# pvjosue/CWFA

Measured on AMD Instinct MI355X. Metric: volumes/sec inverse-pass @512×512×96 fp32; NLL match vs ref (1/2/4/8 GPU), higher is better.
Workload: dtype f32 (storage, accumulation, wavelets, couplings); convolution products on the bf16 matrix cores from an exact three-way bf16 split of both fp32 operands, six products per fp32 product: fp32-equivalent; plain-fp32-MFMA figure: fp32_mfma; 1 GPU; 512x512x96 volume, 4-scale CWFA (CAT blocks, 64 ch) + LRNN inverse, z=0, batch 1/GPU, random-init weights (BASELINE.json configs[2]); precision=split, parallelism=replicated x1 (independent volumes per GPU, no collective)

## Files before the change

### cwfa_amd/_lib.py

```python
import ctypes as C
import os

_HERE = os.path.dirname(os.path.abspath(__file__))
LIB_PATH = os.path.join(_HERE, "libcwfa_hip.so")

CLAMP = {"NONE": 0, "ATAN": 1, "TANH": 2, "SIGMOID": 3}
ACT = {None: 0, "none": 0, "elu": 1, "prelu": 2, "gelu": 3, "relu": 4}
CHAIN_MAX = 8

c_f32p = C.c_void_p
c_i64p = C.c_void_p
c_f64p = C.c_void_p


class AffineStage(C.Structure):
    _fields_ = [("s_raw", c_f32p), ("t", c_f32p), ("s_bs", C.c_int64), ("t_bs", C.c_int64), ("clamp_kind", C.c_int),
                ("clamp", C.c_float), ("pre_scale", C.c_float), ("t_neg_div_sqrt2", C.c_int), ("perm", c_i64p),
                ("perm_axis", C.c_int), ("gin", C.c_int)]


class Chain(C.Structure):
    _fields_ = [("n_stages", C.c_int), ("stage", AffineStage * CHAIN_MAX), ("src_c", C.c_void_p), ("src_h", C.c_void_p)]


class ChainGrads(C.Structure):
    _fields_ = [("ds", c_f32p * CHAIN_MAX), ("dt", c_f32p * CHAIN_MAX), ("ds_bs", C.c_int64 * CHAIN_MAX),
                ("dt_bs", C.c_int64 * CHAIN_MAX)]


class ConvOpts(C.Structure):
    _fields_ = [("bias", c_f32p), ("act", C.c_int), ("prelu_alpha", c_f32p), ("residual", c_f32p), ("res_bs", C.c_int64),
                ("act2", C.c_int), ("in_scale", c_f32p), ("in_shift", c_f32p), ("in_affine_bs", C.c_int), ("in_add", c_f32p),
                ("in_add_bs", C.c_int64), ("upshuffle2", C.c_int), ("in_blocked8", C.c_int), ("out_blocked8", C.c_int),
                ("in_cat", c_f32p), ("in_cat_bs", C.c_int64), ("in_cat_from", C.c_int), ("in_cat_c1", C.c_int), ("out_stats", c_f64p), ("prelu_per_channel", C.c_int),
                ("out_sample_stats", c_f64p)]


class Couple(C.Structure):
    _fields_ = [("x", c_f32p), ("y", c_f32p), ("x_bs", C.c_int64), ("y_bs", C.c_int64), ("n", C.c_int), ("clamp_kind", C.c_int),
                ("clamp", C.c_float), ("pre_scale", C.c_float), ("rev", C.c_int), ("logdet", c_f64p), ("in_blocked8", C.c_int)]


class EvalAffine(C.Structure):
    _fields_ = [("enabled", C.c_int), ("scale", C.c_float), ("std", C.c_float), ("mean", C.c_float)]


class EvalPost(C.Structure):
    _fields_ = [("normalize", C.c_int), ("threshold", C.c_int), ("norm_sub", C.c_float), ("norm_div", C.c_float),
                ("vol_min", C.c_float), ("lower", C.c_float), ("upper", C.c_float), ("clamp_value", C.c_float)]

# ... 244 lines not shown
```

### cwfa_amd/csrc/conv2d.hip

```cpp
#include "conv_internal.h"

#include <string.h>
#include <type_traits>

namespace {

template <int KS_, int CK_, int MT_, int NT_, int WM_, int WN_, int XV_ = 1>
struct Cfg {
    static constexpr int KS = KS_, CK = CK_, MT = MT_, NT = NT_, WM = WM_, WN = WN_;
    static constexpr int XV = XV_;
    static_assert(XV_ == 1 || (XV_ == 4 && KS_ == 1), "vector staging needs halo-free tiles");
    static constexpr int PAD = KS / 2;
    static constexpr int NTHREADS = 64 * WM * WN;
    static constexpr int CT = 32 * MT * WM;
    static constexpr int TR = NT * WN;
    static constexpr int TC = 32;
    static constexpr int XR = TR + KS - 1;
    static constexpr int XC = TC + KS - 1;
    static constexpr int XS = CK * XR * XC;
    static constexpr int XS_PAD = (XS + 3) & ~3;
    static constexpr int WS = KS * KS * CK * CT;
    static constexpr int XPT = (XS / XV + NTHREADS - 1) / NTHREADS;
    static constexpr int WPT = (WS / 4 + NTHREADS - 1) / NTHREADS;
    static constexpr int BUF = XS_PAD + WS;
// ... 195 lines not shown
        chunk_body(chunk & 1, chunk, T{}, F{});
        ++chunk;
    }
    chunk_body(chunk & 1, chunk, F{}, F{});
}

__device__ __forceinline__ float ldg_off(const float* base, unsigned byte_off) {
    asm volatile("" : "+v"(byte_off));
    return *reinterpret_cast<const float*>(reinterpret_cast<const char*>(base) + byte_off);
}
__device__ __forceinline__ void stg_off(float* base, unsigned byte_off, float v) {
    asm volatile("" : "+v"(byte_off));
    *reinterpret_cast<float*>(reinterpret_cast<char*>(base) + byte_off) = v;
}

enum { EPI_GENERIC = 0, EPI_NONE, EPI_ELU, EPI_RES_ELU, EPI_PRELU, EPI_RES_PRELU, EPI_GELU_RES, EPI_UP, EPI_NONE_BLK8, EPI_COUNT };

template <int EPI>
struct EpiTraits {
    static constexpr int ACT1 = EPI == EPI_ELU ? CWFA_ACT_ELU : EPI == EPI_PRELU ? CWFA_ACT_PRELU
                                : EPI == EPI_GELU_RES ? CWFA_ACT_GELU : CWFA_ACT_NONE;
    static constexpr bool RES = EPI == EPI_RES_ELU || EPI == EPI_RES_PRELU || EPI == EPI_GELU_RES;
    static constexpr int ACT2 = EPI == EPI_RES_ELU ? CWFA_ACT_ELU : EPI == EPI_RES_PRELU ? CWFA_ACT_PRELU : CWFA_ACT_NONE;
    static constexpr bool UP = EPI == EPI_UP;
};

template <class C, int EPI>
__device__ __forceinline__ void epilogue(const ConvParams& p, const Tile& t, f32x16 (&acc)[C::MT][C::NT]) {
    typedef EpiTraits<EPI> E;
    const int64_t HW = (int64_t)p.H * p.W;
    const int col = t.col0 + t.l31;
    float* yb = p.y + (int64_t)t.b * p.y_bs;
    if constexpr (EPI == EPI_GENERIC) {
        const float alpha = (p.o.prelu_alpha && (p.o.act == CWFA_ACT_PRELU || p.o.act2 == CWFA_ACT_PRELU)) ? *p.o.prelu_alpha : 0.f;
        const float* rb = p.o.residual ? p.o.residual + (int64_t)t.b * p.o.res_bs : nullptr;
        extern __shared__ __attribute__((aligned(16))) float smem[];
        __syncthreads();
        float* mine = smem + (threadIdx.x >> 6) * 1024 + (threadIdx.x & 63);
        for (int m = 0; m < C::MT; ++m)
// ... 7 lines not shown
                            for (int r = 0; r < 16; ++r) mine[r * 64] = acc[mm][nn][r];
                        }
                const int row = t.row0 + t.wn * C::NT + n;
                for (int r = 0; r < 16; ++r) {
                    const int co = t.ct * C::CT + (t.wm * C::MT + m) * 32 + cwfa_acc_row(r, t.kh);
                    if (co >= p.Cout || row >= p.H || col >= p.W) continue;
                    const int cb = p.o.upshuffle2 ? co >> 2 : co;
                    int64_t o;
                    if (p.o.upshuffle2) {
                        const int q = co & 3;
                        o = (int64_t)cb * (4 * HW) + (int64_t)(2 * row + (q >> 1)) * (2 * p.W) + 2 * col + (q & 1);
                    } else {
                        o = (int64_t)co * HW + (int64_t)row * p.W + col;
                    }
                    float v = cwfa_act(mine[r * 64] + (p.o.bias ? p.o.bias[cb] : 0.f), p.o.act, alpha);
                    if (rb) v += rb[o];
                    yb[o] = cwfa_act(v, p.o.act2, alpha);
                }
            }
    } else {
        float alpha = 0.f;
        if constexpr (E::ACT1 == CWFA_ACT_PRELU || E::ACT2 == CWFA_ACT_PRELU) alpha = *p.o.prelu_alpha;
        const float* rb = nullptr;
        if constexpr (E::RES) rb = p.o.residual + (int64_t)t.b * p.o.res_bs;
        if constexpr (E::UP) {
            const int W2 = 2 * p.W;
            const bool al = ((W2 | (int)(p.y_bs & 1)) & 1) == 0 && ((reinterpret_cast<uintptr_t>(p.y) & 7) == 0);
#pragma unroll
            for (int m = 0; m < C::MT; ++m)
#pragma unroll
                for (int g = 0; g < 4; ++g) {
                    const int co = t.ct * C::CT + (t.wm * C::MT + m) * 32 + 8 * g + 4 * t.kh;
                    if (co >= p.Cout) continue;
                    const int c = co >> 2;
                    const float bias = p.o.bias ? p.o.bias[c] : 0.f;
#pragma unroll
                    for (int n = 0; n < C::NT; ++n) {
                        const int row = t.row0 + t.wn * C::NT + n;
                        if (row >= p.H || col >= p.W) continue;
                        float* o = yb + (int64_t)c * (4 * HW) + (int64_t)(2 * row) * W2 + 2 * col;
                        const float v0 = acc[m][n][4 * g] + bias, v1 = acc[m][n][4 * g + 1] + bias;
                        const float v2 = acc[m][n][4 * g + 2] + bias, v3 = acc[m][n][4 * g + 3] + bias;
                        if (al) {
                            *reinterpret_cast<float2*>(o) = make_float2(v0, v1);
                            *reinterpret_cast<float2*>(o + W2) = make_float2(v2, v3);
                        } else {
                            o[0] = v0; o[1] = v1; o[W2] = v2; o[W2 + 1] = v3;
                        }
                    }
                }
        } else if constexpr (EPI == EPI_NONE_BLK8) {
#pragma unroll
            for (int m = 0; m < C::MT; ++m)
#pragma unroll
                for (int q = 0; q < 4; ++q) {
                    const int co = t.ct * C::CT + (t.wm * C::MT + m) * 32 + 8 * q + 4 * t.kh;
                    if (co >= p.Cout) continue;
                    const f32x4 b4 = p.o.bias ? *reinterpret_cast<const f32x4*>(p.o.bias + co) : f32x4{0.f, 0.f, 0.f, 0.f};
#pragma unroll
                    for (int n = 0; n < C::NT; ++n) {
                        const int row = t.row0 + t.wn * C::NT + n;
                        if (row >= p.H || col >= p.W) continue;
                        f32x4 v;
#pragma unroll
                        for (int i = 0; i < 4; ++i) v[i] = acc[m][n][4 * q + i] + b4[i];
// ... 167 lines not shown
struct Sel {
    int id, CT, CK;
};

Sel select_cfg(int ks, int Cout) {
    const int cls = Cout <= 32 ? 0 : (Cout <= 64 ? 1 : 2);
    if (ks == 3) return cls == 0 ? Sel{0, C3_32::CT, C3_32::CK} : cls == 1 ? Sel{1, C3_64::CT, C3_64::CK} : Sel{2, C3_128::CT, C3_128::CK};
    if (ks == 1) return cls == 0 ? Sel{3, C1_32::CT, C1_32::CK} : cls == 1 ? Sel{4, C1_64::CT, C1_64::CK} : Sel{5, C1_128::CT, C1_128::CK};
    if (ks == 7) return cls == 0 ? Sel{6, C7_32::CT, C7_32::CK} : Sel{7, C7_64::CT, C7_64::CK};
    return Sel{-1, 0, 0};
}

int classify_epilogue(const cwfa_conv_opts& o) {
    const bool res = o.residual != nullptr;
    if (o.out_blocked8) return EPI_NONE_BLK8;
    if (o.upshuffle2) return (!res && o.act == CWFA_ACT_NONE && o.act2 == CWFA_ACT_NONE) ? EPI_UP : EPI_GENERIC;
    if (!res && o.act2 == CWFA_ACT_NONE) {
        if (o.act == CWFA_ACT_NONE) return EPI_NONE;
        if (o.act == CWFA_ACT_ELU) return EPI_ELU;
        if (o.act == CWFA_ACT_PRELU) return EPI_PRELU;
    }
    if (res && o.act == CWFA_ACT_NONE && o.act2 == CWFA_ACT_ELU) return EPI_RES_ELU;
    if (res && o.act == CWFA_ACT_NONE && o.act2 == CWFA_ACT_PRELU) return EPI_RES_PRELU;
    if (res && o.act == CWFA_ACT_GELU && o.act2 == CWFA_ACT_NONE) return EPI_GELU_RES;
    return EPI_GENERIC;
}

template <class C>
int prepare(ConvParams& p, dim3& grid) {
    p.tiles_x = (p.W + C::TC - 1) / C::TC;
    p.tiles_y = (p.H + C::TR - 1) / C::TR;
// ... 19 lines not shown
    CWFA_LAUNCH_CHECK("cwfa_conv2d_f32");
    return CWFA_OK;
}

template <class C, unsigned ALLOWED, bool PRO>
int launch_sel(const ConvParams& p, int epi, hipStream_t st) {
    if (!(ALLOWED & (1u << epi)) && epi != EPI_NONE_BLK8) epi = EPI_GENERIC;
    switch (epi) {
        case EPI_NONE: if constexpr (ALLOWED & (1u << EPI_NONE)) return launch_epi<C, EPI_NONE, PRO>(p, st); break;
        case EPI_ELU: if constexpr (ALLOWED & (1u << EPI_ELU)) return launch_epi<C, EPI_ELU, PRO>(p, st); break;
        case EPI_RES_ELU: if constexpr (ALLOWED & (1u << EPI_RES_ELU)) return launch_epi<C, EPI_RES_ELU, PRO>(p, st); break;
        case EPI_PRELU: if constexpr (ALLOWED & (1u << EPI_PRELU)) return launch_epi<C, EPI_PRELU, PRO>(p, st); break;
        case EPI_RES_PRELU: if constexpr (ALLOWED & (1u << EPI_RES_PRELU)) return launch_epi<C, EPI_RES_PRELU, PRO>(p, st); break;
        case EPI_GELU_RES: if constexpr (ALLOWED & (1u << EPI_GELU_RES)) return launch_epi<C, EPI_GELU_RES, PRO>(p, st); break;
        case EPI_UP: if constexpr (ALLOWED & (1u << EPI_UP)) return launch_epi<C, EPI_UP, PRO>(p, st); break;
        case EPI_NONE_BLK8:
            if constexpr (ALLOWED & (1u << EPI_NONE_BLK8)) return launch_epi<C, EPI_NONE_BLK8, PRO>(p, st);
            cwfa_set_error("cwfa_conv2d_f32: out_blocked8 is built for the 1x1 kernels with more than 32 output channels");
            return CWFA_E_SHAPE;
        default: break;
    }
    return launch_epi<C, EPI_GENERIC, PRO>(p, st);
}

template <class C, unsigned ALLOWED, unsigned ALLOWED_PRO>
int launch(const ConvParams& p, int epi, hipStream_t st) {
    if (p.o.in_scale || p.o.in_add) return launch_sel<C, ALLOWED_PRO, true>(p, epi, st);
    return launch_sel<C, ALLOWED, false>(p, epi, st);
}

// ... 6 lines not shown

int fill_params(ConvParams& p, const char* name, const float* x, const float* w_packed, float* y, int B, int Cin, int H,
                int W, int Cout, int64_t x_bs, int64_t y_bs, const cwfa_conv_opts* opts) {
    CWFA_REQUIRE(B >= 0 && Cin > 0 && Cout > 0 && H >= 0 && W >= 0, CWFA_E_INVAL, "%s: bad size", name);
    if (B == 0 || H == 0 || W == 0) return 1;
    CWFA_REQUIRE(x && w_packed && y, CWFA_E_INVAL, "%s: null pointer", name);
    CWFA_REQUIRE(!opts || !opts->out_sample_stats, CWFA_E_INVAL, "%s: out_sample_stats is a feature of the few-channel cwfa_conv7x7_split_f32", name);
    CWFA_REQUIRE((int64_t)Cin * H * W < (1ll << 30) && (int64_t)Cout * H * W * (p.o.upshuffle2 ? 1 : 1) < (1ll << 30), CWFA_E_SHAPE, "%s: C*H*W exceeds the 32-bit byte offsets of a tile (2^30 elements per image)", name);
    CWFA_REQUIRE(cwfa_aligned16(w_packed), CWFA_E_ALIGN, "%s: packed weights must be 16-byte aligned", name);
    p.x = x; p.wp = w_packed; p.y = y;
    p.B = B; p.Cin = Cin; p.H = H; p.W = W; p.Cout = Cout;
    p.x_bs = x_bs; p.y_bs = y_bs;
    p.products = g_cwfa_operand == CwfaOperand::split3 ? 6 : 1;
    if (opts) p.o = *opts;
    CWFA_REQUIRE(!(p.o.in_scale && !p.o.in_shift), CWFA_E_INVAL, "%s: in_scale without in_shift", name);
    CWFA_REQUIRE(p.o.act >= 0 && p.o.act <= CWFA_ACT_RELU && p.o.act2 >= 0 && p.o.act2 <= CWFA_ACT_RELU, CWFA_E_INVAL,
                 "%s: bad activation", name);
    CWFA_REQUIRE(!((p.o.act == CWFA_ACT_PRELU || p.o.act2 == CWFA_ACT_PRELU) && !p.o.prelu_alpha), CWFA_E_INVAL,
                 "%s: PReLU without prelu_alpha", name);
    return CWFA_OK;
}

typedef Cfg<1, 16, 2, 4, 4, 2> CS;
constexpr int CS_XB = 3 * 2 * 8 * 32 * 16, CS_WB = 3 * 2 * 256 * 16, CS_BUFB = CS_XB + CS_WB;

__device__ __forceinline__ void split3(float v, unsigned short (&o)[3]) {
    const __bf16 a1 = (__bf16)v;
    const float r1 = v - (float)a1;
    const __bf16 a2 = (__bf16)r1;
    const float r2 = r1 - (float)a2;
// ... 263 lines not shown
    ConvParams& p = sp.c;
    CWFA_REQUIRE(!p.o.in_scale && !p.o.in_add, CWFA_E_INVAL, "cwfa_conv_split_f32: the load-side prologue belongs in cwfa_split_input_f32");
    CWFA_REQUIRE(!p.o.upshuffle2 || (ks == 1 && Cout % 4 == 0), CWFA_E_SHAPE, "cwfa_conv_split_f32: upshuffle2 needs ks=1, Cout=4*Co");
    CWFA_REQUIRE(!p.o.out_stats && !p.o.prelu_per_channel, CWFA_E_INVAL, "cwfa_conv_split_f32: out_stats / prelu_per_channel are features of cwfa_conv3x3_split_f32");
    p.nchunks = (Cin + 15) / 16;
    sp.ws = ws;
    sp.CG2 = 2 * p.nchunks;
    sp.ws_bs = (int64_t)3 * sp.CG2 * H * W * 16;
    CWFA_REQUIRE(sp.ws_bs + (int64_t)4 * H * W * 16 < (1ll << 31) && (int64_t)(p.nchunks * ks * ks + 2) * CS_WB < (1ll << 31), CWFA_E_SHAPE,
                 "cwfa_conv_split_f32: one sample's planes / one cout tile's weights must stay below 2 GiB");
    const int epi = classify_epilogue(p.o);
    hipStream_t st = (hipStream_t)stream;
    switch (epi) {
        case EPI_NONE: return launch_split<EPI_NONE>(sp, st);
        case EPI_UP: return launch_split<EPI_UP>(sp, st);
        default: return launch_split<EPI_GENERIC>(sp, st);
    }
}

int g_cwfa_wino_min_cout = 1;
int g_cwfa_wino_2d = 512;
CwfaOperand g_cwfa_operand = CwfaOperand::split3;

extern "C" int cwfa_set_option(const char* name, int value) {
    CWFA_REQUIRE(name, CWFA_E_INVAL, "cwfa_set_option: null name");
    if (strcmp(name, "winograd_min_cout") == 0) {
        g_cwfa_wino_min_cout = value;
        return CWFA_OK;
    }
    if (strcmp(name, "winograd_2d") == 0) {
// ... 80 lines not shown
    CWFA_REQUIRE(!(opts && opts->out_blocked8) || (ks == 1 && Cout % 8 == 0 && !opts->residual && opts->act == CWFA_ACT_NONE &&
                                                   opts->act2 == CWFA_ACT_NONE && !opts->upshuffle2 && !opts->in_scale && !opts->in_add &&
                                                   cwfa_aligned16(y) && (y_bs & 3) == 0 && (!opts->bias || cwfa_aligned16(opts->bias))),
                 CWFA_E_INVAL, "cwfa_conv2d_f32: out_blocked8 needs a plain 1x1 bank (bias only), Cout %% 8 == 0 and 16-byte aligned y / bias");
    const Sel s = select_cfg(ks, Cout);
    CWFA_REQUIRE(s.id >= 0, CWFA_E_SHAPE, "cwfa_conv2d_f32: kernel size %d not in {1,3,7}", ks);
    ConvParams p{};
    int rc = fill_params(p, "cwfa_conv2d_f32", x, w_packed, y, B, Cin, H, W, Cout, x_bs, y_bs, opts);
    if (rc) return rc < 0 ? rc : CWFA_OK;
    CWFA_REQUIRE(!p.o.upshuffle2 || (ks == 1 && Cout % 4 == 0), CWFA_E_SHAPE, "cwfa_conv2d_f32: upshuffle2 needs ks=1, Cout=4*Co");
    CWFA_REQUIRE(!p.o.out_stats && !p.o.prelu_per_channel, CWFA_E_INVAL, "cwfa_conv2d_f32: out_stats / prelu_per_channel are features of cwfa_conv3x3_split_f32");
    const int epi = classify_epilogue(p.o);
    hipStream_t st = (hipStream_t)stream;
    if (cwfa_wino_selected(ks, Cout)) return cwfa_wino_conv(x, w_packed, y, B, Cin, H, W, Cout, x_bs, y_bs, p.o, st);
    constexpr unsigned N = 1u << EPI_NONE, E = 1u << EPI_ELU, RE = 1u << EPI_RES_ELU, P = 1u << EPI_PRELU,
                       RP = 1u << EPI_RES_PRELU, G = 1u << EPI_GELU_RES, U = 1u << EPI_UP, K = 1u << EPI_NONE_BLK8;
    const bool v4 = ks == 1 && (W & 3) == 0 && (x_bs & 3) == 0 && (reinterpret_cast<uintptr_t>(x) & 15) == 0 &&
                    (!p.o.in_add || ((p.o.in_add_bs & 3) == 0 && (reinterpret_cast<uintptr_t>(p.o.in_add) & 15) == 0));
    if (v4) {
        switch (s.id) {
            case 3: return launch<C1v_32, N | P | G, P>(p, epi, st);
            case 4: return launch<C1v_64, N | RE | G | K, 0>(p, epi, st);
            default: return launch<C1v_128, N | U | K, U>(p, epi, st);
        }
    }
    switch (s.id) {
        case 0: return launch<C3_32, N | P | RP, 0>(p, epi, st);
        case 1: return launch<C3_64, N | E | P | RP, 0>(p, epi, st);
        case 2: return launch<C3_128, N | P, P>(p, epi, st);
        case 3: return launch<C1_32, N | P | G, P>(p, epi, st);
        case 4: return launch<C1_64, N | RE | G | K, 0>(p, epi, st);
        case 5: return launch<C1_128, N | U | K, U>(p, epi, st);
        case 6: return launch<C7_32, N, 0>(p, epi, st);
        default: return launch<C7_64, N, 0>(p, epi, st);
    }
}

extern "C" int cwfa_subnet_pack1x1_f32(const float* w, float* panel, void* stream) {
    CWFA_REQUIRE(w && panel, CWFA_E_INVAL, "cwfa_subnet_pack1x1_f32: null pointer");
    hipLaunchKernelGGL(pack1x1_kernel, dim3(16), dim3(256), 0, (hipStream_t)stream, w, panel);
    CWFA_LAUNCH_CHECK("cwfa_subnet_pack1x1_f32");
    return CWFA_OK;
}

extern "C" int cwfa_subnet_layer_tape_f32(const float* x, const float* w3_packed, const float* b3, const float* w1_panel,
                                          const float* b1, float* y, float* hidden, int B, int H, int W, int64_t x_bs, int64_t y_bs,
                                          int64_t hidden_bs, void* stream) {
// ... 36 lines not shown
```

### cwfa_amd/csrc/conv_split3x3.hip

```cpp
#include "conv_internal.h"

extern int g_cwfa_split_xcd_map;
extern int g_cwfa_split_rows16;

namespace {

constexpr int TR = 8, TC = 32;

template <int KS, int RPW = 4>
struct XG {
    static constexpr int TRW = 2 * RPW, NT = 2 * RPW;
    static constexpr int PAD = KS / 2, XR = TRW + 2 * PAD, XC = TC + 2 * PAD, NTAP = KS * KS;
    static constexpr int EPK = XR * XC;
    static constexpr int KHB = KS == 7 ? 8512 : RPW == 8 ? 9792 : 5440;
    static constexpr int XPB = 2 * KHB;
    static constexpr int XB = 3 * XPB;
    static constexpr bool SPECIAL = KS == 3 && RPW == 4;
    static constexpr int NEK = SPECIAL ? 2 : 3;
    static_assert(EPK * 16 <= KHB && KHB % 256 == 64 && 2 * EPK <= 512 * NEK, "staging entry map");
    static_assert(!SPECIAL || (EPK > 256 && EPK <= 384), "3x3 staging entry map");
    static_assert(KS == 3 || RPW == 4, "7x7: 8-row tiles");
};

template <int MPW, int KS = 3, int RPW = 4, int WM = 4>
// ... 856 lines not shown
    pack_bank(w, packed, Cout, Cin, ct_of(Cout), 9, (hipStream_t)stream);
    CWFA_LAUNCH_CHECK("cwfa_conv3x3_split_pack_f32");
    return CWFA_OK;
}

extern "C" int cwfa_conv3x3_split_f32(const float* x, const void* w_packed, float* y, int B, int Cin, int H, int W, int Cout,
                                      int64_t x_bs, int64_t y_bs, const cwfa_conv_opts* opts, void* stream) {
    CWFA_REQUIRE(B >= 0 && Cin > 0 && Cout > 0 && H >= 0 && W >= 0, CWFA_E_INVAL, "cwfa_conv3x3_split_f32: bad size");
    if (B == 0 || H == 0 || W == 0) return CWFA_OK;
    CWFA_REQUIRE(x && w_packed && y, CWFA_E_INVAL, "cwfa_conv3x3_split_f32: null pointer");
    CWFA_REQUIRE(cwfa_aligned16(w_packed), CWFA_E_ALIGN, "cwfa_conv3x3_split_f32: packed weights must be 16-byte aligned");
    SParams p{};
    p.x = x; p.wp = w_packed; p.y = y;
    p.B = B; p.Cin = Cin; p.H = H; p.W = W; p.Cout = Cout; p.x_bs = x_bs; p.y_bs = y_bs;
    if (opts) p.o = *opts;
    CWFA_REQUIRE(!p.o.upshuffle2 && !p.o.in_cat, CWFA_E_SHAPE, "cwfa_conv3x3_split_f32: upshuffle2 / in_cat are 1x1 features");
    CWFA_REQUIRE(!p.o.out_sample_stats, CWFA_E_INVAL, "cwfa_conv3x3_split_f32: out_sample_stats is a feature of the few-channel cwfa_conv7x7_split_f32");
    CWFA_REQUIRE(!p.o.in_blocked8 || (Cin % 8 == 0 && cwfa_aligned16(x) && (x_bs & 3) == 0 && !p.o.in_add), CWFA_E_ALIGN,
                 "cwfa_conv3x3_split_f32: blocked input needs Cin %% 8 == 0, 16-byte alignment and no added tensor");
    CWFA_REQUIRE(!p.o.out_blocked8 || (Cout % 8 == 0 && cwfa_aligned16(y) && (y_bs & 3) == 0 && !p.o.residual && p.o.act2 == CWFA_ACT_NONE &&
                                       (p.o.act == CWFA_ACT_NONE || p.o.act == CWFA_ACT_PRELU)),
                 CWFA_E_ALIGN, "cwfa_conv3x3_split_f32: blocked output needs Cout %% 8 == 0, 16-byte alignment and a bias / PReLU epilogue");
    CWFA_REQUIRE(!(p.o.in_scale && !p.o.in_shift), CWFA_E_INVAL, "cwfa_conv3x3_split_f32: in_scale without in_shift");
    CWFA_REQUIRE(!p.o.out_stats || (!p.o.out_blocked8 && !p.o.residual && p.o.act2 == CWFA_ACT_NONE &&
                                    (p.o.act == CWFA_ACT_NONE || p.o.act == CWFA_ACT_PRELU)),
                 CWFA_E_INVAL, "cwfa_conv3x3_split_f32: out_stats needs an NCHW output and a bias / PReLU epilogue");
    CWFA_REQUIRE(!((p.o.out_stats || p.o.out_blocked8) && p.o.in_add && p.o.act == CWFA_ACT_NONE), CWFA_E_INVAL,
                 "cwfa_conv3x3_split_f32: out_stats / out_blocked8 with in_add need a PReLU epilogue");
    CWFA_REQUIRE(p.o.act >= 0 && p.o.act <= CWFA_ACT_RELU && p.o.act2 >= 0 && p.o.act2 <= CWFA_ACT_RELU, CWFA_E_INVAL,
                 "cwfa_conv3x3_split_f32: bad activation");
    CWFA_REQUIRE(!((p.o.act == CWFA_ACT_PRELU || p.o.act2 == CWFA_ACT_PRELU) && !p.o.prelu_alpha), CWFA_E_INVAL,
// ... 99 lines not shown
```

### cwfa_amd/ops.py

```python
import ctypes as C
from collections import namedtuple

import torch

from . import _lib
from ._lib import AffineStage, Chain, ConvOpts, check

__all__ = ["haar1d", "haar2d", "gather", "affine", "channel_affine", "chain_inv", "chain_inv_var", "chain_inv_roi_cov", "chain_inv_samples", "rand_uniform", "rand_trunc_normal", "rand_poisson", "chain_nll_map", "nll_compose", "chain_fwd", "pack_conv_weight",
           "conv2d", "conv2d_wgrad", "elu_bwd", "set_precision", "gelu_add", "gelu_bwd", "layernorm_bwd", "attention_bwd", "plane_affine", "bn_bwd_stats", "bn_act_bwd", "maxpool2_bwd", "chain_bwd", "chain_inv_bwd", "prelu_bwd", "conv3d_1k1_backward", "pack_1x1_panel", "pack_split_layer_weight", "subnet_layer", "conv3d_1k1", "channel_stats", "bn_fold", "bn_running_update", "maxpool", "sample_stats", "layernorm_apply",
           "convnext_tail", "conv_writes_sample_stats", "attention_combine", "scale_channels", "axpby", "stage", "lion_step", "global_extrema", "wmse_loss"]


def _stream():
    return C.c_void_p(torch.cuda.current_stream().cuda_stream)


def _p(t):
    return None if t is None else C.c_void_p(t.data_ptr())


def _dev(t, name="tensor"):
    if not torch.is_tensor(t):
        raise TypeError(f"{name}: expected a torch.Tensor, got {type(t)}")
    if not t.is_cuda:
# ... 600 lines not shown
    pc.version, pc.src_ptr = w._version, w.data_ptr()
    pc.cat_c1, pc.cat_from = c1, start
    return pc


def conv_writes_stats(pc, act=None, residual=None, act2=None, out_blocked=False, in_add=False):
    return bool(pc.split and pc.ks == 3 and act in (None, "prelu") and residual is None and act2 is None and not out_blocked
                and not (in_add and act is None))


def conv_writes_sample_stats(pc):
    return bool(pc.split and pc.ks == 7 and pc.cin <= 8)


def conv2d(x, pc, bias=None, act=None, prelu_alpha=None, residual=None, act2=None, in_scale=None, in_shift=None,
           in_add=None, out=None, in_blocked=False, out_blocked=False, cat=None, out_stats=None, out_sample_stats=None):
    L = _lib.lib()
    x, xbs = planes(x, "x")
    B, Cin, H, W = x.shape
    o = ConvOpts()
    keep = [x]
    walk = out_walk_selected(pc, H, W, act=act, prelu_alpha=prelu_alpha, residual=residual, act2=act2, in_scale=in_scale, in_add=in_add,
                             out_blocked=out_blocked, cat=cat, out_stats=out_stats, out_sample_stats=out_sample_stats)
    if cat is not None:
        cat, cbs = planes(cat, "cat")
        c1 = getattr(pc, "cat_c1", None)
        if c1 is None or Cin != c1 or tuple(cat.shape) != (B, pc.cin - pc.cat_from, H, W) or in_scale is not None or in_add is not None:
            raise ValueError("conv2d: `cat` needs a bank from pack_conv_weight_cat for exactly these two inputs, and no load-side prologue")
        o.in_cat, o.in_cat_bs, o.in_cat_from, o.in_cat_c1 = cat.data_ptr(), cbs, pc.cat_from, c1
        keep.append(cat)
        Cin = pc.cin
# ... 16 lines not shown
    if prelu_alpha is not None:
        prelu_alpha = _dev(prelu_alpha, "prelu_alpha")
        o.prelu_alpha = prelu_alpha.data_ptr()
        if prelu_alpha.numel() != 1:
            if prelu_alpha.numel() != pc.cout or not prelu_alpha.is_contiguous() or not (pc.split and pc.ks == 3):
                raise ValueError("conv2d: per-channel PReLU slopes need [Cout] contiguous values and the split-bf16 3x3 kernel")
            o.prelu_per_channel = 1
    elif "prelu" in (act, act2):
        raise ValueError("conv2d: PReLU needs prelu_alpha")
    if residual is not None:
        residual, rbs = planes(residual, "residual")
        if tuple(residual.shape) != oshape:
            raise ValueError(f"conv2d: residual {tuple(residual.shape)} != output {oshape}")
        o.residual, o.res_bs = residual.data_ptr(), rbs
        keep.append(residual)
    if in_scale is not None:
        o.in_scale, o.in_shift = _dev(in_scale).data_ptr(), _dev(in_shift).data_ptr()
        if in_scale.numel() not in (Cin, B * Cin) or in_shift.numel() != in_scale.numel():
            raise ValueError("conv2d: in_scale / in_shift must be [Cin] or [B,Cin]")
        o.in_affine_bs = Cin if (in_scale.numel() == B * Cin and B > 1) else 0
    if in_add is not None:
        in_add, abs_ = planes(in_add, "in_add")
        if tuple(in_add.shape) != tuple(x.shape):
            raise ValueError("conv2d: in_add shape mismatch")
        o.in_add, o.in_add_bs = in_add.data_ptr(), abs_
        keep.append(in_add)
    o.upshuffle2 = int(up)
    if in_blocked:
        if not (walk or (pc.split and pc.ks == 3)):
            raise ValueError("conv2d: channel-blocked input is read by the split-bf16 3x3 kernels only")
# ... 117 lines not shown
        if rec.want(key):
            e0, e1 = torch.cuda.Event(enable_timing=True), torch.cuda.Event(enable_timing=True)
            e0.record()
    check(L.cwfa_conv3x3_split_couple_f32(_p(u), _p(pc.packed), _p(br), B, Cin, H, W, ubs, C.byref(cp), _stream()),
          "conv3x3_split_couple")
    if rec is not None and rec.want(key):
        e1.record()
        rec.add(key, e0, e1)
    return out


BLOCKED_MAPS = True
SPLIT_7X7 = True
VIRTUAL_CAT = True
COUPLE_EPILOGUE = True


def couple_fused():
    return COUPLE_EPILOGUE and _split_bf16 >= 2


def split3x3_narrow(cout):
    return cout <= 48 or 64 < cout <= 96


SPLIT_3X3_MIN_COUT = 1
SPLIT_3X3_NARROW_MAX = 16
OUT_WALK = True
OUT_WALK_MT = (1, 2, 3)

# ... 2543 lines not shown
```

### cwfa_amd/unet.py

```python
import torch
from torch import nn

from . import ops
from .amp import amp_entry

__all__ = ["UNet", "UNetConvBlock", "UNetUpBlock"]


_MATERIALIZE_UP = False
_MATERIALIZE = True


class _Packed:

    def __init__(self):
        self._c = {}

    def get(self, conv, transposed=False):
        w = conv.weight
        pc = self._c.get(id(conv))
        if pc is None or pc.version != w._version or pc.src_ptr != w.data_ptr() or pc.epoch != ops.pack_epoch():
            pc = self._c[id(conv)] = ops.pack_conv_weight(w, transposed=transposed)
        return pc

# ... 159 lines not shown
        in_size = out_size if not skip_conn else in_size // 2
        self.conv_block = UNetConvBlock(in_size, out_size, padding, batch_norm, use_bias=use_bias, activation=activation)
        self._packed = _Packed()

    @staticmethod
    def center_crop(layer, target_size):
        _, _, h, w = layer.size()
        dy, dx = (h - target_size[0]) // 2, (w - target_size[1]) // 2
        return layer[:, :, dy:(dy + target_size[0]), dx:(dx + target_size[1])]

    def run(self, x, bridge, in_affine=None, out_mask=None):
        sc, sh = in_affine if in_affine is not None else (None, None)
        if _MATERIALIZE_UP and ops._split_bf16 < 1 and sc is not None and (x.shape[2] * x.shape[3]) % 4 == 0:
            x = ops.plane_affine(x, sc, sh)
            sc = sh = None
        up = ops.conv2d(x, self._packed.get(self.up, transposed=True), bias=self.up.bias, in_scale=sc, in_shift=sh)
        add = self.center_crop(bridge, up.shape[2:]) if self.skip_conn else None
        return self.conv_block.run(up, in_add=add, out_mask=out_mask)

    @amp_entry
    def forward(self, x, bridge):
        y, aff = self.run(x, bridge)
        return y if aff is None else ops.channel_affine(y, aff[0], aff[1])


class UNet(nn.Module):

    def __init__(self, in_channels=1, n_classes=2, depth=5, wf=6, padding=True, batch_norm=True, up_mode='upsample',
                 drop_out=0, use_bias=False, skip_conn=False, activation=nn.PReLU):
        super().__init__()
        assert up_mode in ('upconv', 'upsample')
# ... 15 lines not shown
    @amp_entry
    def forward(self, x, store_activations=False, in_affine=None):
        if store_activations:
            raise NotImplementedError("store_activations is a debugging aid of the reference, not on the hot path")
        B, dev = x.shape[0], x.device
        skips, aff = [], in_affine
        n_draw = 0
        if self.drop_out:
            n_draw = B * (sum(d.block[0].out_channels for d in list(self.down_path)[:-1]) +
                          sum(u.conv_block.block[0].out_channels for u in self.up_path))
        pool = _DrawPool(n_draw, dev)
        for i, down in enumerate(self.down_path):
            x, aff = down.run(x, in_affine=aff)
            if i != len(self.down_path) - 1:
                sc, sh = aff if aff is not None else (None, None)
                x, full = ops.maxpool(x, x.shape[-1] // 2, x.shape[-1] // 2, sc, sh, want_full=True)
                skips.append(full)
                m = _drop(self.drop_out, B, x.shape[1], dev, pool)
                aff = _drop_affine(x.shape[1], m) if m is not None else None
        for i, up in enumerate(self.up_path):
            m = _drop(self.drop_out, B, up.conv_block.block[0].out_channels, dev, pool)
            x, aff = up.run(x, skips[-i - 1], in_affine=aff, out_mask=m)
        kind, alpha = UNetConvBlock._act(self.last[1])
        sc, sh = aff if aff is not None else (None, None)
        return ops.conv2d(x, self._packed.get(self.last[0]), bias=self.last[0].bias, act=kind, prelu_alpha=alpha,
                          in_scale=sc, in_shift=sh)
```

### include/cwfa_hip.h

```cpp
#ifndef CWFA_HIP_H
#define CWFA_HIP_H

#include <stdint.h>

#ifdef __cplusplus
extern "C" {
#endif

#define CWFA_VERSION 100

enum {
    CWFA_OK = 0,
    CWFA_E_INVAL = -1,
    CWFA_E_SHAPE = -2,
    CWFA_E_ALIGN = -3,
    CWFA_E_HIP = -4
};

enum { CWFA_CLAMP_NONE = 0, CWFA_CLAMP_ATAN = 1, CWFA_CLAMP_TANH = 2, CWFA_CLAMP_SIGMOID = 3 };

enum { CWFA_ACT_NONE = 0, CWFA_ACT_ELU = 1, CWFA_ACT_PRELU = 2, CWFA_ACT_GELU = 3, CWFA_ACT_RELU = 4 };

int cwfa_version(void);
const char* cwfa_last_error(void);
// ... 97 lines not shown
    int act2;
    const float* in_scale;
    const float* in_shift;
    int in_affine_bs;
    const float* in_add;
    int64_t in_add_bs;
    int upshuffle2;
    int in_blocked8;
    int out_blocked8;
    const float* in_cat;
    int64_t in_cat_bs;
    int in_cat_from, in_cat_c1;
    double* out_stats;
    int prelu_per_channel;
    double* out_sample_stats;
} cwfa_conv_opts;

int cwfa_conv2d_f32(const float* x, const float* w_packed, float* y, int B, int Cin, int H, int W, int Cout, int ks,
                    int64_t x_bs, int64_t y_bs, const cwfa_conv_opts* opts, void* stream);

int cwfa_subnet_pack1x1_f32(const float* w, float* panel, void* stream);
int cwfa_subnet_layer_f32(const float* x, const float* w3_packed, const float* b3, const float* w1_panel, const float* b1,
                          float* y, int B, int H, int W, int64_t x_bs, int64_t y_bs, void* stream);
int cwfa_subnet_layer_tape_f32(const float* x, const float* w3_packed, const float* b3, const float* w1_panel, const float* b1,
                               float* y, float* hidden, int B, int H, int W, int64_t x_bs, int64_t y_bs, int64_t hidden_bs,
                               void* stream);

int cwfa_conv3d_1k1_f32(const float* x, const float* w1, const float* b1, const float* alpha, const float* w2,
                        const float* b2, float* y, int B, int D, int H, int W, int K, void* stream);
int cwfa_conv3d_1k1_split_f32(const float* x, const float* w1, const float* b1, const float* alpha, const float* w2,
// ... 332 lines not shown
```

Before: 57.49 volumes/s.

## Fuse UNet skip connection into transposed-conv upshuffle epilogue with affine residual

Instead of materializing the affine-applied full skip tensor during maxpool and then adding it as in_add at the up block's conv, the down path now stores the raw pre-pool tensor plus its pending affine. The up-path transposed 1x1 conv adds that residual (with per-channel scale/shift applied) directly in a new EPI_UP_RES epilogue using vectorized float2 loads. This removes one full-resolution write and a later read of the skip tensor at each scale. The cost is extra residual loads in the epilogue, more register pressure, and a new ABI field in the conv options struct.

Result: no change. 57.99 volumes/s, median of 6 (+0.9%).

```diff
diff --git a/cwfa_amd/_lib.py b/cwfa_amd/_lib.py
--- a/cwfa_amd/_lib.py
+++ b/cwfa_amd/_lib.py
@@ -33,7 +33,7 @@
                 ("act2", C.c_int), ("in_scale", c_f32p), ("in_shift", c_f32p), ("in_affine_bs", C.c_int), ("in_add", c_f32p),
                 ("in_add_bs", C.c_int64), ("upshuffle2", C.c_int), ("in_blocked8", C.c_int), ("out_blocked8", C.c_int),
                 ("in_cat", c_f32p), ("in_cat_bs", C.c_int64), ("in_cat_from", C.c_int), ("in_cat_c1", C.c_int), ("out_stats", c_f64p), ("prelu_per_channel", C.c_int),
-                ("out_sample_stats", c_f64p)]
+                ("out_sample_stats", c_f64p), ("res_scale", c_f32p), ("res_shift", c_f32p), ("res_affine_bs", C.c_int)]
 
 
 class Couple(C.Structure):
diff --git a/cwfa_amd/csrc/conv2d.hip b/cwfa_amd/csrc/conv2d.hip
--- a/cwfa_amd/csrc/conv2d.hip
+++ b/cwfa_amd/csrc/conv2d.hip
@@ -233,7 +233,12 @@
     *reinterpret_cast<float*>(reinterpret_cast<char*>(base) + byte_off) = v;
 }
 
-enum { EPI_GENERIC = 0, EPI_NONE, EPI_ELU, EPI_RES_ELU, EPI_PRELU, EPI_RES_PRELU, EPI_GELU_RES, EPI_UP, EPI_NONE_BLK8, EPI_COUNT };
+__device__ __forceinline__ float2 ldg2_off(const float* base, unsigned byte_off) {
+    asm volatile("" : "+v"(byte_off));
+    return *reinterpret_cast<const float2*>(reinterpret_cast<const char*>(base) + byte_off);
+}
+
+enum { EPI_GENERIC = 0, EPI_NONE, EPI_ELU, EPI_RES_ELU, EPI_PRELU, EPI_RES_PRELU, EPI_GELU_RES, EPI_UP, EPI_NONE_BLK8, EPI_UP_RES, EPI_COUNT };
 
 template <int EPI>
 struct EpiTraits {
@@ -241,7 +246,8 @@
                                 : EPI == EPI_GELU_RES ? CWFA_ACT_GELU : CWFA_ACT_NONE;
     static constexpr bool RES = EPI == EPI_RES_ELU || EPI == EPI_RES_PRELU || EPI == EPI_GELU_RES;
     static constexpr int ACT2 = EPI == EPI_RES_ELU ? CWFA_ACT_ELU : EPI == EPI_RES_PRELU ? CWFA_ACT_PRELU : CWFA_ACT_NONE;
-    static constexpr bool UP = EPI == EPI_UP;
+    static constexpr bool UP = EPI == EPI_UP || EPI == EPI_UP_RES;
+    static constexpr bool UP_RES = EPI == EPI_UP_RES;
 };
 
 template <class C, int EPI>
@@ -279,7 +285,14 @@
                         o = (int64_t)co * HW + (int64_t)row * p.W + col;
                     }
                     float v = cwfa_act(mine[r * 64] + (p.o.bias ? p.o.bias[cb] : 0.f), p.o.act, alpha);
-                    if (rb) v += rb[o];
+                    if (rb) {
+                        float r = rb[o];
+                        if (p.o.res_scale) {
+                            const int64_t a = (int64_t)t.b * p.o.res_affine_bs + cb;
+                            r = r * p.o.res_scale[a] + p.o.res_shift[a];
+                        }
+                        v += r;
+                    }
                     yb[o] = cwfa_act(v, p.o.act2, alpha);
                 }
             }
@@ -287,12 +300,51 @@
         float alpha = 0.f;
         if constexpr (E::ACT1 == CWFA_ACT_PRELU || E::ACT2 == CWFA_ACT_PRELU) alpha = *p.o.prelu_alpha;
         const float* rb = nullptr;
-        if constexpr (E::RES) rb = p.o.residual + (int64_t)t.b * p.o.res_bs;
+        if constexpr (E::RES || E::UP_RES) rb = p.o.residual + (int64_t)t.b * p.o.res_bs;
         if constexpr (E::UP) {
             const int W2 = 2 * p.W;
             const bool al = ((W2 | (int)(p.y_bs & 1)) & 1) == 0 && ((reinterpret_cast<uintptr_t>(p.y) & 7) == 0);
 #pragma unroll
-            for (int m = 0; m < C::MT; ++m)
+            for (int m = 0; m < C::MT; ++m) {
+                [[maybe_unused]] float2 res[E::UP_RES ? 4 : 1][E::UP_RES ? C::NT : 1][2];
+                if constexpr (E::UP_RES) {
+                    const bool ral = (p.o.res_bs & 1) == 0 && (reinterpret_cast<uintptr_t>(p.o.residual) & 7) == 0;
+                    const int colc = col < p.W ? col : p.W - 1;
+                    float rsc[4], rsh[4];
+#pragma unroll
+                    for (int g = 0; g < 4; ++g) {
+                        int c = (t.ct * C::CT + (t.wm * C::MT + m) * 32 + 8 * g + 4 * t.kh) >> 2;
+                        c = c < (p.Cout >> 2) ? c : (p.Cout >> 2) - 1;
+                        if (p.o.res_scale) {
+                            rsc[g] = p.o.res_scale[(int64_t)t.b * p.o.res_affine_bs + c];
+                            rsh[g] = p.o.res_shift[(int64_t)t.b * p.o.res_affine_bs + c];
+                        }
+#pragma unroll
+                        for (int n = 0; n < C::NT; ++n) {
+                            int row = t.row0 + t.wn * C::NT + n;
+                            row = row < p.H ? row : p.H - 1;
+                            const unsigned off = ((unsigned)c * (unsigned)(4 * HW) + (unsigned)(2 * row) * (unsigned)W2 + 2u * (unsigned)colc) * 4u;
+                            if (ral) {
+                                res[g][n][0] = ldg2_off(rb, off);
+                                res[g][n][1] = ldg2_off(rb, off + 4u * (unsigned)W2);
+                            } else {
+                                res[g][n][0] = make_float2(ldg_off(rb, off), ldg_off(rb, off + 4u));
+                                res[g][n][1] = make_float2(ldg_off(rb, off + 4u * (unsigned)W2), ldg_off(rb, off + 4u * (unsigned)W2 + 4u));
+                            }
+                        }
+                    }
+                    if (p.o.res_scale) {
+#pragma unroll
+                        for (int g = 0; g < 4; ++g)
+#pragma unroll
+                            for (int n = 0; n < C::NT; ++n)
+#pragma unroll
+                                for (int k = 0; k < 2; ++k) {
+                                    res[g][n][k].x = res[g][n][k].x * rsc[g] + rsh[g];
+                                    res[g][n][k].y = res[g][n][k].y * rsc[g] + rsh[g];
+                                }
+                    }
+                }
 #pragma unroll
                 for (int g = 0; g < 4; ++g) {
                     const int co = t.ct * C::CT + (t.wm * C::MT + m) * 32 + 8 * g + 4 * t.kh;
@@ -304,8 +356,12 @@
                         const int row = t.row0 + t.wn * C::NT + n;
                         if (row >= p.H || col >= p.W) continue;
                         float* o = yb + (int64_t)c * (4 * HW) + (int64_t)(2 * row) * W2 + 2 * col;
-                        const float v0 = acc[m][n][4 * g] + bias, v1 = acc[m][n][4 * g + 1] + bias;
-                        const float v2 = acc[m][n][4 * g + 2] + bias, v3 = acc[m][n][4 * g + 3] + bias;
+                        float v0 = acc[m][n][4 * g] + bias, v1 = acc[m][n][4 * g + 1] + bias;
+                        float v2 = acc[m][n][4 * g + 2] + bias, v3 = acc[m][n][4 * g + 3] + bias;
+                        if constexpr (E::UP_RES) {
+                            v0 += res[g][n][0].x; v1 += res[g][n][0].y;
+                            v2 += res[g][n][1].x; v3 += res[g][n][1].y;
+                        }
                         if (al) {
                             *reinterpret_cast<float2*>(o) = make_float2(v0, v1);
                             *reinterpret_cast<float2*>(o + W2) = make_float2(v2, v3);
@@ -314,6 +370,7 @@
                         }
                     }
                 }
+            }
         } else if constexpr (EPI == EPI_NONE_BLK8) {
 #pragma unroll
             for (int m = 0; m < C::MT; ++m)
@@ -511,7 +568,7 @@
 int classify_epilogue(const cwfa_conv_opts& o) {
     const bool res = o.residual != nullptr;
     if (o.out_blocked8) return EPI_NONE_BLK8;
-    if (o.upshuffle2) return (!res && o.act == CWFA_ACT_NONE && o.act2 == CWFA_ACT_NONE) ? EPI_UP : EPI_GENERIC;
+    if (o.upshuffle2) return (o.act != CWFA_ACT_NONE || o.act2 != CWFA_ACT_NONE) ? EPI_GENERIC : res ? EPI_UP_RES : EPI_UP;
     if (!res && o.act2 == CWFA_ACT_NONE) {
         if (o.act == CWFA_ACT_NONE) return EPI_NONE;
         if (o.act == CWFA_ACT_ELU) return EPI_ELU;
@@ -561,6 +618,7 @@
         case EPI_RES_PRELU: if constexpr (ALLOWED & (1u << EPI_RES_PRELU)) return launch_epi<C, EPI_RES_PRELU, PRO>(p, st); break;
         case EPI_GELU_RES: if constexpr (ALLOWED & (1u << EPI_GELU_RES)) return launch_epi<C, EPI_GELU_RES, PRO>(p, st); break;
         case EPI_UP: if constexpr (ALLOWED & (1u << EPI_UP)) return launch_epi<C, EPI_UP, PRO>(p, st); break;
+        case EPI_UP_RES: if constexpr (ALLOWED & (1u << EPI_UP_RES)) return launch_epi<C, EPI_UP_RES, PRO>(p, st); break;
         case EPI_NONE_BLK8:
             if constexpr (ALLOWED & (1u << EPI_NONE_BLK8)) return launch_epi<C, EPI_NONE_BLK8, PRO>(p, st);
             cwfa_set_error("cwfa_conv2d_f32: out_blocked8 is built for the 1x1 kernels with more than 32 output channels");
@@ -597,6 +655,8 @@
     p.products = g_cwfa_operand == CwfaOperand::split3 ? 6 : 1;
     if (opts) p.o = *opts;
     CWFA_REQUIRE(!(p.o.in_scale && !p.o.in_shift), CWFA_E_INVAL, "%s: in_scale without in_shift", name);
+    CWFA_REQUIRE(!p.o.res_scale == !p.o.res_shift && (!p.o.res_scale || (p.o.residual && p.o.upshuffle2)), CWFA_E_INVAL,
+                 "%s: res_scale and res_shift go together, with the residual of an upshuffle2 bank", name);
     CWFA_REQUIRE(p.o.act >= 0 && p.o.act <= CWFA_ACT_RELU && p.o.act2 >= 0 && p.o.act2 <= CWFA_ACT_RELU, CWFA_E_INVAL,
                  "%s: bad activation", name);
     CWFA_REQUIRE(!((p.o.act == CWFA_ACT_PRELU || p.o.act2 == CWFA_ACT_PRELU) && !p.o.prelu_alpha), CWFA_E_INVAL,
@@ -890,6 +950,7 @@
     switch (epi) {
         case EPI_NONE: return launch_split<EPI_NONE>(sp, st);
         case EPI_UP: return launch_split<EPI_UP>(sp, st);
+        case EPI_UP_RES: return launch_split<EPI_UP_RES>(sp, st);
         default: return launch_split<EPI_GENERIC>(sp, st);
     }
 }
@@ -1000,14 +1061,14 @@
     hipStream_t st = (hipStream_t)stream;
     if (cwfa_wino_selected(ks, Cout)) return cwfa_wino_conv(x, w_packed, y, B, Cin, H, W, Cout, x_bs, y_bs, p.o, st);
     constexpr unsigned N = 1u << EPI_NONE, E = 1u << EPI_ELU, RE = 1u << EPI_RES_ELU, P = 1u << EPI_PRELU,
-                       RP = 1u << EPI_RES_PRELU, G = 1u << EPI_GELU_RES, U = 1u << EPI_UP, K = 1u << EPI_NONE_BLK8;
+                       RP = 1u << EPI_RES_PRELU, G = 1u << EPI_GELU_RES, U = 1u << EPI_UP, K = 1u << EPI_NONE_BLK8, UR = 1u << EPI_UP_RES;
     const bool v4 = ks == 1 && (W & 3) == 0 && (x_bs & 3) == 0 && (reinterpret_cast<uintptr_t>(x) & 15) == 0 &&
                     (!p.o.in_add || ((p.o.in_add_bs & 3) == 0 && (reinterpret_cast<uintptr_t>(p.o.in_add) & 15) == 0));
     if (v4) {
         switch (s.id) {
             case 3: return launch<C1v_32, N | P | G, P>(p, epi, st);
             case 4: return launch<C1v_64, N | RE | G | K, 0>(p, epi, st);
-            default: return launch<C1v_128, N | U | K, U>(p, epi, st);
+            default: return launch<C1v_128, N | U | UR | K, U | UR>(p, epi, st);
         }
     }
     switch (s.id) {
@@ -1016,7 +1077,7 @@
         case 2: return launch<C3_128, N | P, P>(p, epi, st);
         case 3: return launch<C1_32, N | P | G, P>(p, epi, st);
         case 4: return launch<C1_64, N | RE | G | K, 0>(p, epi, st);
-        case 5: return launch<C1_128, N | U | K, U>(p, epi, st);
+        case 5: return launch<C1_128, N | U | UR | K, U | UR>(p, epi, st);
         case 6: return launch<C7_32, N, 0>(p, epi, st);
         default: return launch<C7_64, N, 0>(p, epi, st);
     }
diff --git a/cwfa_amd/csrc/conv_split3x3.hip b/cwfa_amd/csrc/conv_split3x3.hip
--- a/cwfa_amd/csrc/conv_split3x3.hip
+++ b/cwfa_amd/csrc/conv_split3x3.hip
@@ -894,7 +894,8 @@
     p.x = x; p.wp = w_packed; p.y = y;
     p.B = B; p.Cin = Cin; p.H = H; p.W = W; p.Cout = Cout; p.x_bs = x_bs; p.y_bs = y_bs;
     if (opts) p.o = *opts;
-    CWFA_REQUIRE(!p.o.upshuffle2 && !p.o.in_cat, CWFA_E_SHAPE, "cwfa_conv3x3_split_f32: upshuffle2 / in_cat are 1x1 features");
+    CWFA_REQUIRE(!p.o.upshuffle2 && !p.o.in_cat && !p.o.res_scale && !p.o.res_shift, CWFA_E_SHAPE,
+                 "cwfa_conv3x3_split_f32: upshuffle2 / in_cat / res_scale are 1x1 features");
     CWFA_REQUIRE(!p.o.out_sample_stats, CWFA_E_INVAL, "cwfa_conv3x3_split_f32: out_sample_stats is a feature of the few-channel cwfa_conv7x7_split_f32");
     CWFA_REQUIRE(!p.o.in_blocked8 || (Cin % 8 == 0 && cwfa_aligned16(x) && (x_bs & 3) == 0 && !p.o.in_add), CWFA_E_ALIGN,
                  "cwfa_conv3x3_split_f32: blocked input needs Cin %% 8 == 0, 16-byte alignment and no added tensor");
diff --git a/cwfa_amd/ops.py b/cwfa_amd/ops.py
--- a/cwfa_amd/ops.py
+++ b/cwfa_amd/ops.py
@@ -638,7 +638,8 @@
 
 
 def conv2d(x, pc, bias=None, act=None, prelu_alpha=None, residual=None, act2=None, in_scale=None, in_shift=None,
-           in_add=None, out=None, in_blocked=False, out_blocked=False, cat=None, out_stats=None, out_sample_stats=None):
+           in_add=None, out=None, in_blocked=False, out_blocked=False, cat=None, out_stats=None, out_sample_stats=None,
+           res_scale=None, res_shift=None):
     L = _lib.lib()
     x, xbs = planes(x, "x")
     B, Cin, H, W = x.shape
@@ -685,6 +686,16 @@
             raise ValueError(f"conv2d: residual {tuple(residual.shape)} != output {oshape}")
         o.residual, o.res_bs = residual.data_ptr(), rbs
         keep.append(residual)
+    if res_scale is not None or res_shift is not None:
+        if not up or residual is None or res_scale is None or res_shift is None:
+            raise ValueError("conv2d: res_scale / res_shift go together, with the residual of a transposed bank")
+        Co = oshape[1]
+        res_scale, res_shift = _dev(res_scale, "res_scale").contiguous(), _dev(res_shift, "res_shift").contiguous()
+        if res_scale.numel() not in (Co, B * Co) or res_shift.numel() != res_scale.numel():
+            raise ValueError("conv2d: res_scale / res_shift must be [Co] or [B,Co]")
+        o.res_scale, o.res_shift = res_scale.data_ptr(), res_shift.data_ptr()
+        o.res_affine_bs = Co if (res_scale.numel() == B * Co and B > 1) else 0
+        keep += [res_scale, res_shift]
     if in_scale is not None:
         o.in_scale, o.in_shift = _dev(in_scale).data_ptr(), _dev(in_shift).data_ptr()
         if in_scale.numel() not in (Cin, B * Cin) or in_shift.numel() != in_scale.numel():
@@ -832,6 +843,7 @@
 SPLIT_7X7 = True
 VIRTUAL_CAT = True
 COUPLE_EPILOGUE = True
+SKIP_AT_UP = True
 
 
 def couple_fused():
diff --git a/cwfa_amd/unet.py b/cwfa_amd/unet.py
--- a/cwfa_amd/unet.py
+++ b/cwfa_amd/unet.py
@@ -197,7 +197,18 @@
         if _MATERIALIZE_UP and ops._split_bf16 < 1 and sc is not None and (x.shape[2] * x.shape[3]) % 4 == 0:
             x = ops.plane_affine(x, sc, sh)
             sc = sh = None
-        up = ops.conv2d(x, self._packed.get(self.up, transposed=True), bias=self.up.bias, in_scale=sc, in_shift=sh)
+        pc = self._packed.get(self.up, transposed=True)
+        if isinstance(bridge, tuple):
+            raw, raff = bridge
+            rsc, rsh = raff if raff is not None else (None, None)
+            oshape = (x.shape[0], pc.cout // 4, 2 * x.shape[2], 2 * x.shape[3])
+            if self.skip_conn and tuple(raw.shape) == oshape and ops.planes(raw)[0] is raw:
+                up = ops.conv2d(x, pc, bias=self.up.bias, in_scale=sc, in_shift=sh, residual=raw, res_scale=rsc, res_shift=rsh)
+                return self.conv_block.run(up, out_mask=out_mask)
+            bridge = None
+            if self.skip_conn:
+                bridge = raw if rsc is None else ops.maxpool(raw, raw.shape[-2] // 2, raw.shape[-1] // 2, rsc, rsh, want_full=True)[1]
+        up = ops.conv2d(x, pc, bias=self.up.bias, in_scale=sc, in_shift=sh)
         add = self.center_crop(bridge, up.shape[2:]) if self.skip_conn else None
         return self.conv_block.run(up, in_add=add, out_mask=out_mask)
 
@@ -243,8 +254,12 @@
             x, aff = down.run(x, in_affine=aff)
             if i != len(self.down_path) - 1:
                 sc, sh = aff if aff is not None else (None, None)
-                x, full = ops.maxpool(x, x.shape[-1] // 2, x.shape[-1] // 2, sc, sh, want_full=True)
-                skips.append(full)
+                if ops.SKIP_AT_UP and self.skip_conn:
+                    skips.append((x, aff))
+                    x = ops.maxpool(x, x.shape[-1] // 2, x.shape[-1] // 2, sc, sh, want_full=False)
+                else:
+                    x, full = ops.maxpool(x, x.shape[-1] // 2, x.shape[-1] // 2, sc, sh, want_full=True)
+                    skips.append(full)
                 m = _drop(self.drop_out, B, x.shape[1], dev, pool)
                 aff = _drop_affine(x.shape[1], m) if m is not None else None
         for i, up in enumerate(self.up_path):
diff --git a/include/cwfa_hip.h b/include/cwfa_hip.h
--- a/include/cwfa_hip.h
+++ b/include/cwfa_hip.h
@@ -135,6 +135,9 @@
     double* out_stats;
     int prelu_per_channel;
     double* out_sample_stats;
+    const float* res_scale;
+    const float* res_shift;
+    int res_affine_bs;
 } cwfa_conv_opts;
 
 int cwfa_conv2d_f32(const float* x, const float* w_packed, float* y, int B, int Cin, int H, int W, int Cout, int ks,
```
